# cassianobecker/tgcn

Hardware: AMD Instinct MI355X
Metric: Cheb-TGCN fwd: G edge·timesteps/s + achieved HBM GB/s, K=5 on 160M-edge graph (higher is better)
Workload: dtype f32

## Files before the change

### tgcn_amd/csrc/common.h

```cpp
#pragma once


thread_local char g_err[512] = "";

#define TGCN_FAIL(code, ...)                    \
  do {                                          \
    snprintf(g_err, sizeof(g_err), __VA_ARGS__); \
    return (code);                              \
  } while (0)

#define TGCN_CHECK_LAUNCH(what)                                                         \
  do {                                                                                  \
    hipError_t e_ = hipGetLastError();                                                  \
    if (e_ != hipSuccess) TGCN_FAIL(TGCN_ERR_LAUNCH, "%s: %s", what, hipGetErrorString(e_)); \
  } while (0)

constexpr int kBlock = 256;

struct ProfRec { hipEvent_t a, b; int kind; };
thread_local std::vector<ProfRec> g_prof;
thread_local int g_prof_cap = 0;

struct ProfScope {
  hipEvent_t b = nullptr;
// ... 30 lines not shown
  if (hipGetDevice(&dev) != hipSuccess || dev < 0 || dev >= 16) return 64 * 1024;
  int v = cached[dev].load(std::memory_order_relaxed);
  if (v > 0) return v;
  if (hipDeviceGetAttribute(&v, hipDeviceAttributeSharedMemPerBlockOptin, dev) != hipSuccess || v <= 0) {
    (void)hipGetLastError();
    if (hipDeviceGetAttribute(&v, hipDeviceAttributeMaxSharedMemoryPerBlock, dev) != hipSuccess || v <= 0) v = 64 * 1024;
  }
  cached[dev].store(v, std::memory_order_relaxed);
  return v;
}

inline int cu_count() {
  static std::atomic<int> cached[16];
  int dev = 0;
  if (hipGetDevice(&dev) != hipSuccess || dev < 0 || dev >= 16) return 256;
  int v = cached[dev].load(std::memory_order_relaxed);
  if (v > 0) return v;
  if (hipDeviceGetAttribute(&v, hipDeviceAttributeMultiprocessorCount, dev) != hipSuccess || v <= 0) v = 256;
  cached[dev].store(v, std::memory_order_relaxed);
  return v;
}

struct TuneInt {
  int v;
  int load() const { return v; }
  void store(int x) { v = x; }
};
thread_local TuneInt g_hop_variant{0};
thread_local TuneInt g_hop_remap{1};
thread_local TuneInt g_hop_seg_remap{0};
thread_local TuneInt g_hop_mix{0};
thread_local TuneInt g_hop_stream{1};
thread_local TuneInt g_hop_lds_pad{0};
thread_local TuneInt g_proj_variant{0};
thread_local TuneInt g_x3_form{2};
thread_local TuneInt g_x3_tail{1};
thread_local TuneInt g_small_narrow{1};
thread_local TuneInt g_small_dense{2};
thread_local TuneInt g_x3_stream_cap{0};
thread_local TuneInt g_overlap{1};
thread_local TuneInt g_overlap_group{3};
thread_local TuneInt g_overlap_min_mb{256};

struct SideStream {
  hipStream_t st = nullptr;
  hipEvent_t ev[4] = {nullptr, nullptr, nullptr, nullptr};
  int next = 0;
  hipEvent_t event() { hipEvent_t e = ev[next]; next = (next + 1) & 3; return e; }
};
thread_local std::map<int, SideStream>* g_side = nullptr;
thread_local int64_t g_side_launches = 0;

inline SideStream* side_stream() {
  int dev = 0;
  if (hipGetDevice(&dev) != hipSuccess) return nullptr;
  if (!g_side) g_side = new std::map<int, SideStream>();
  SideStream& s = (*g_side)[dev];
  if (s.st) return &s;
  int least = 0, greatest = 0;
  if (hipDeviceGetStreamPriorityRange(&least, &greatest) != hipSuccess) { (void)hipGetLastError(); least = 0; }
  for (auto& e : s.ev)
    if (!e && hipEventCreateWithFlags(&e, hipEventDisableTiming) != hipSuccess) { (void)hipGetLastError(); e = nullptr; return nullptr; }
  if (hipStreamCreateWithPriority(&s.st, hipStreamNonBlocking, least) != hipSuccess) { (void)hipGetLastError(); s.st = nullptr; return nullptr; }
  return &s;
}

// ... 17 lines not shown
```

### tgcn_amd/csrc/device_build.h

```cpp
#pragma once

constexpr int kScanPer = 8;
constexpr int kScanTile = kBlock * kScanPer;

__global__ __launch_bounds__(kBlock) void scan_tile_kernel(const int64_t* in, int64_t* out,
                                                           int64_t* __restrict__ tile_sums, int64_t n, int inclusive) {
  __shared__ int64_t wave_tot[kBlock / 64];
  const int tid = threadIdx.x, lane = tid & 63, wave = tid >> 6;
  const int64_t base = (int64_t)blockIdx.x * kScanTile + (int64_t)tid * kScanPer;
  int64_t v[kScanPer];
  int64_t run = 0;
#pragma unroll
  for (int j = 0; j < kScanPer; ++j) {
    v[j] = (base + j < n) ? in[base + j] : 0;
    run += v[j];
  }
  int64_t inc = run;
#pragma unroll
  for (int off = 1; off < 64; off <<= 1) {
    const int64_t t = __shfl_up(inc, off, 64);
    if (lane >= off) inc += t;
  }
  if (lane == 63) wave_tot[wave] = inc;
  __syncthreads();
// ... 350 lines not shown
                     1.401298464324817e-45f , dis);
  const int64_t total = m + (diag ? n : 0);
  if (total > 0)
    hipLaunchKernelGGL(lap_values_kernel, dim3(grid_1d(total)), dim3(kBlock), 0, st, row, col, w, m, n, (const float*)dis, scale, diag, row_out, col_out, val_out);
  TGCN_CHECK_LAUNCH("adjacency_normalise");
  *count_host = total;
  return TGCN_OK;
}

__global__ void sched_cost_kernel(const int32_t* __restrict__ rowptr, int64_t n, int row_thresh, int wave_max, int row_cost, int64_t* __restrict__ cost,
                                  int64_t* __restrict__ is_seg, int64_t* __restrict__ is_wave, unsigned long long* __restrict__ n_empty) {
  unsigned long long mine = 0;
  for (int64_t i = (int64_t)blockIdx.x * blockDim.x + threadIdx.x; i < n; i += (int64_t)gridDim.x * blockDim.x) {
    const int64_t d = rowptr[i + 1] - rowptr[i];
    cost[i] = (d > row_thresh ? 0 : d) + row_cost;
    is_seg[i] = d > wave_max ? 1 : 0;
    is_wave[i] = (d > row_thresh && d <= wave_max) ? 1 : 0;
    mine += (d == 0);
  }
  if (mine) atomicAdd(n_empty, mine);
}

__global__ void sched_marks_kernel(const int64_t* __restrict__ cum, int64_t n, int64_t target, int64_t nblk, int32_t* __restrict__ blk_row) {
  for (int64_t b = (int64_t)blockIdx.x * blockDim.x + threadIdx.x; b <= nblk; b += (int64_t)gridDim.x * blockDim.x) {
    if (b == 0) { blk_row[0] = 0; continue; }
    if (b == nblk) { blk_row[nblk] = (int32_t)n; continue; }
    const int64_t mark = b * target;
    int64_t lo = 0, hi = n;
    while (lo < hi) { const int64_t mid = (lo + hi) >> 1; if (cum[mid] < mark) lo = mid + 1; else hi = mid; }
    blk_row[b] = (int32_t)((lo + 1 < n) ? lo + 1 : n);
  }
}

__global__ void sched_longrows_kernel(const int32_t* __restrict__ rowptr, int64_t n, const int64_t* __restrict__ is_seg,
                                      const int64_t* __restrict__ pos, int seg_len, uint32_t max_key, uint32_t* __restrict__ seg_rows,
                                      uint32_t* __restrict__ key) {
  for (int64_t i = (int64_t)blockIdx.x * blockDim.x + threadIdx.x; i < n; i += (int64_t)gridDim.x * blockDim.x) {
    if (!is_seg[i]) continue;
    const int64_t d = rowptr[i + 1] - rowptr[i];
    const int64_t o = pos[i];
    seg_rows[o] = (uint32_t)i;
    key[o] = max_key - (uint32_t)((d + seg_len - 1) / seg_len);
  }
}

__global__ void sched_waverows_kernel(const int32_t* __restrict__ rowptr, const tgcn_edge* __restrict__ edges, int64_t n, const int64_t* __restrict__ is_wave,
                                      const int64_t* __restrict__ pos, uint32_t* __restrict__ rows, uint32_t* __restrict__ key) {
  for (int64_t i = (int64_t)blockIdx.x * blockDim.x + threadIdx.x; i < n; i += (int64_t)gridDim.x * blockDim.x) {
    if (!is_wave[i]) continue;
    const int64_t o = pos[i];
    rows[o] = (uint32_t)i;
    key[o] = (uint32_t)edges[rowptr[i]].col;
  }
}

__global__ void sched_wavesegs_kernel(const int32_t* __restrict__ rowptr, const uint32_t* __restrict__ rows, int64_t nw, int32_t* __restrict__ seg_row,
                                      int32_t* __restrict__ seg_e0, int32_t* __restrict__ seg_e1, int32_t* __restrict__ seg_slot) {
  for (int64_t i = (int64_t)blockIdx.x * blockDim.x + threadIdx.x; i < nw; i += (int64_t)gridDim.x * blockDim.x) {
    const int64_t r = rows[i];
    seg_row[i] = (int32_t)r; seg_e0[i] = rowptr[r]; seg_e1[i] = rowptr[r + 1]; seg_slot[i] = -1;
  }
}

__global__ void sched_nsegs_kernel(const uint32_t* __restrict__ key, uint32_t max_key, int64_t m, int64_t* __restrict__ nsegs) {
  for (int64_t i = (int64_t)blockIdx.x * blockDim.x + threadIdx.x; i < m; i += (int64_t)gridDim.x * blockDim.x) nsegs[i] = max_key - key[i];
}

__global__ void sched_segments_kernel(const int32_t* __restrict__ rowptr, const tgcn_edge* __restrict__ edges, const uint32_t* __restrict__ seg_rows,
                                      const int64_t* __restrict__ first, int64_t m, int64_t nseg, int64_t npartial, int seg_len,
                                      int32_t* __restrict__ seg_row, int32_t* __restrict__ seg_e0, int32_t* __restrict__ seg_e1,
                                      int32_t* __restrict__ seg_slot, uint32_t* __restrict__ key, uint32_t* __restrict__ ident) {
  for (int64_t s = (int64_t)blockIdx.x * blockDim.x + threadIdx.x; s < nseg; s += (int64_t)gridDim.x * blockDim.x) {
    int64_t lo = 0, hi = m;
    while (lo + 1 < hi) { const int64_t mid = (lo + hi) >> 1; if (first[mid] <= s) lo = mid; else hi = mid; }
    const int64_t r = seg_rows[lo];
    const int64_t e0 = (int64_t)rowptr[r] + (s - first[lo]) * seg_len;
    const int64_t e1 = (e0 + seg_len < (int64_t)rowptr[r + 1]) ? e0 + seg_len : (int64_t)rowptr[r + 1];
    seg_row[s] = (int32_t)r;
    seg_e0[s] = (int32_t)e0;
    seg_e1[s] = (int32_t)e1;
    seg_slot[s] = s < npartial ? (int32_t)s : -1;
    key[s] = (uint32_t)edges[e0].col;
    ident[s] = (uint32_t)s;
  }
}

__global__ void permute_i32_kernel(const int32_t* __restrict__ in, const uint32_t* __restrict__ perm, int32_t* __restrict__ out, int64_t n) {
  for (int64_t i = (int64_t)blockIdx.x * blockDim.x + threadIdx.x; i < n; i += (int64_t)gridDim.x * blockDim.x) out[i] = in[perm[i]];
}

__global__ void sched_long_kernel(const uint32_t* __restrict__ seg_rows, const int64_t* __restrict__ first, int64_t nlong, int64_t npartial,
                                  int32_t* __restrict__ long_row, int32_t* __restrict__ long_slot) {
  for (int64_t i = (int64_t)blockIdx.x * blockDim.x + threadIdx.x; i <= nlong; i += (int64_t)gridDim.x * blockDim.x) {
    if (i < nlong) { long_row[i] = (int32_t)seg_rows[i]; long_slot[i] = (int32_t)first[i]; }
    else long_slot[nlong] = (int32_t)npartial;
  }
}

__global__ void sched_counts_kernel(const int64_t* __restrict__ nsegs, int64_t m, int huge_slots, int64_t* __restrict__ out2) {
  if (blockIdx.x != 0 || threadIdx.x != 0) return;
  for (int which = 0; which < 2; ++which) {
    const int64_t thr = which == 0 ? 1 : huge_slots;
    int64_t lo = 0, hi = m;
    while (lo < hi) { const int64_t mid = (lo + hi) >> 1; if (nsegs[mid] > thr) lo = mid + 1; else hi = mid; }
    out2[which] = lo;
  }
}
```

### tgcn_amd/csrc/graph_build.h

```cpp
#pragma once

struct DeviceBuf {
  void* p = nullptr;
  ~DeviceBuf() { if (p) (void)hipFree(p); }
  int alloc(size_t bytes) {
    if (p) { (void)hipFree(p); p = nullptr; }
    if (hipMalloc(&p, bytes ? bytes : 16) != hipSuccess) { p = nullptr; return -1; }
    return 0;
  }
  int zero(size_t bytes) { return (alloc(bytes) || hipMemset(p, 0, bytes ? bytes : 16) != hipSuccess) ? -1 : 0; }
};

}

struct tgcn_graph {
  tgcn_csr csr;
  int64_t n_cols;
  DeviceBuf rowptr, edges;
};

struct tgcn_sched {
  tgcn_csr_sched s;
  DeviceBuf blk_row, seg_row, seg_e0, seg_e1, seg_slot, long_row, long_slot;
};
// ... 125 lines not shown

int tgcn_sched_build_csr(const tgcn_csr* A, int64_t n_cols, int32_t C, int aligned16, tgcn_sched** out) {
  if (!A || !out || C <= 0 || A->n <= 0 || !A->rowptr || (A->nnz > 0 && !A->edges) || n_cols <= 0) TGCN_FAIL(TGCN_ERR_INVALID, "sched_build: bad argument");
  const int lanes = hop_geom(C, aligned16).lpr;
  const int gpb = kBlock / lanes;
  const int64_t n = A->n;
  const int32_t seg_mode = 0;
  const int32_t row_thresh = 32, seg_len = 32, huge_slots = 64, row_cost = 4;
  const int64_t max_blocks_hint = 2048;
  hipStream_t st = (hipStream_t)0;
  tgcn_sched* sc = new (std::nothrow) tgcn_sched();
  if (!sc) TGCN_FAIL(TGCN_ERR_LAUNCH, "sched_build: out of host memory");
#define TGCN_SCHED_FAIL(...) do { delete sc; TGCN_FAIL(TGCN_ERR_LAUNCH, __VA_ARGS__); } while (0)
  const int32_t wave_max = lanes == 16 ? 32 * (64 / lanes) : row_thresh;
  DeviceBuf cost, is_seg, is_wave, pos, posw, scanws, empties;
  if (empties.zero(8) || cost.alloc((size_t)n * 8) || is_seg.zero((size_t)(n + 1) * 8) || is_wave.zero((size_t)(n + 1) * 8) || pos.alloc((size_t)(n + 1) * 8) ||
      posw.alloc((size_t)(n + 1) * 8) || scanws.alloc(scan_ws_elems(n + 1) * 8))
    TGCN_SCHED_FAIL("sched_build: device allocation failed");
  hipLaunchKernelGGL(sched_cost_kernel, dim3(grid_1d(n)), dim3(kBlock), 0, st, A->rowptr, n, (int)row_thresh, (int)wave_max, (int)row_cost, (int64_t*)cost.p,
                     (int64_t*)is_seg.p, (int64_t*)is_wave.p, (unsigned long long*)empties.p);
  scan_i64(st, (const int64_t*)cost.p, (int64_t*)cost.p, n, 1, (int64_t*)scanws.p);
  scan_i64(st, (const int64_t*)is_seg.p, (int64_t*)pos.p, n + 1, 0, (int64_t*)scanws.p);
  scan_i64(st, (const int64_t*)is_wave.p, (int64_t*)posw.p, n + 1, 0, (int64_t*)scanws.p);
  int64_t total = 0, m = 0, mw = 0, n_empty = 0;
  if (read_back(&total, (const int64_t*)cost.p + (n - 1)) || read_back(&m, (const int64_t*)pos.p + n) || read_back(&mw, (const int64_t*)posw.p + n) ||
      read_back(&n_empty, (const int64_t*)empties.p))
    TGCN_SCHED_FAIL("sched_build: device read failed");
  const int64_t cap = lanes <= 16 ? 64 : 256;
  const int64_t target = std::max<int64_t>(gpb * 16, std::min<int64_t>(gpb * cap, (total + max_blocks_hint - 1) / max_blocks_hint));
  const int64_t nblk = std::max<int64_t>(1, (total + target - 1) / target);
  if (sc->blk_row.alloc((size_t)(nblk + 1) * 4)) TGCN_SCHED_FAIL("sched_build: device allocation failed");
  hipLaunchKernelGGL(sched_marks_kernel, dim3(grid_1d(nblk + 1)), dim3(kBlock), 0, st, (const int64_t*)cost.p, n, target, nblk, (int32_t*)sc->blk_row.p);
  int64_t nlong = 0, nhuge = 0, npartial = 0, nsegl = 0;
  DeviceBuf seg_rows, key, sortws, nsegs, first, cnt2;
  if (m > 0) {
    const uint32_t max_key = (uint32_t)((A->nnz + seg_len - 1) / seg_len + 1);
    if (seg_rows.alloc((size_t)m * 4) || key.alloc((size_t)m * 4) || sortws.alloc(sort_ws_bytes(m)) || nsegs.zero((size_t)(m + 1) * 8) ||
        first.alloc((size_t)(m + 1) * 8) || cnt2.alloc(16))
      TGCN_SCHED_FAIL("sched_build: device allocation failed");
    hipLaunchKernelGGL(sched_longrows_kernel, dim3(grid_1d(n)), dim3(kBlock), 0, st, A->rowptr, n, (const int64_t*)is_seg.p, (const int64_t*)pos.p,
                       (int)seg_len, max_key, (uint32_t*)seg_rows.p, (uint32_t*)key.p);
    radix_sort_pairs(st, (uint32_t*)key.p, (uint32_t*)seg_rows.p, m, bits_for((int64_t)max_key + 1), (char*)sortws.p);
    hipLaunchKernelGGL(sched_nsegs_kernel, dim3(grid_1d(m)), dim3(kBlock), 0, st, (const uint32_t*)key.p, max_key, m, (int64_t*)nsegs.p);
    hipLaunchKernelGGL(sched_counts_kernel, dim3(1), dim3(64), 0, st, (const int64_t*)nsegs.p, m, (int)huge_slots, (int64_t*)cnt2.p);
    scan_i64(st, (const int64_t*)nsegs.p, (int64_t*)first.p, m + 1, 0, (int64_t*)scanws.p);
    int64_t h2[2] = {0, 0};
    if (hipMemcpy(h2, cnt2.p, 16, hipMemcpyDeviceToHost) != hipSuccess || read_back(&nsegl, (const int64_t*)first.p + m)) TGCN_SCHED_FAIL("sched_build: device read failed");
    nlong = h2[0]; nhuge = h2[1];
    if (nlong > 0 && read_back(&npartial, (const int64_t*)first.p + nlong)) TGCN_SCHED_FAIL("sched_build: device read failed");
  }
  const int64_t nseg = mw + nsegl;
  if (nseg >= (int64_t)INT32_MAX) TGCN_SCHED_FAIL("sched_build: too many segments");
  const size_t sball = (size_t)(nseg > 0 ? nseg : 1) * 4;
  if (sc->seg_row.zero(sball) || sc->seg_e0.zero(sball) || sc->seg_e1.zero(sball) || sc->seg_slot.zero(sball) || sc->long_row.zero((size_t)(nlong ? nlong : 1) * 4) ||
      sc->long_slot.zero((size_t)(nlong + 2) * 4))
    TGCN_SCHED_FAIL("sched_build: device allocation failed");
  DeviceBuf wrows, wkey, wsort, u_row, u_e0, u_e1, u_slot, key2, ident, sortws2;
  if (mw > 0) {
    if (wrows.alloc((size_t)mw * 4) || wkey.alloc((size_t)mw * 4) || wsort.alloc(sort_ws_bytes(mw))) TGCN_SCHED_FAIL("sched_build: device allocation failed");
    hipLaunchKernelGGL(sched_waverows_kernel, dim3(grid_1d(n)), dim3(kBlock), 0, st, A->rowptr, A->edges, n, (const int64_t*)is_wave.p, (const int64_t*)posw.p,
                       (uint32_t*)wrows.p, (uint32_t*)wkey.p);
    radix_sort_pairs(st, (uint32_t*)wkey.p, (uint32_t*)wrows.p, mw, bits_for(n_cols), (char*)wsort.p);
    hipLaunchKernelGGL(sched_wavesegs_kernel, dim3(grid_1d(mw)), dim3(kBlock), 0, st, A->rowptr, (const uint32_t*)wrows.p, mw, (int32_t*)sc->seg_row.p,
                       (int32_t*)sc->seg_e0.p, (int32_t*)sc->seg_e1.p, (int32_t*)sc->seg_slot.p);
  }
  if (nsegl > 0) {
    const size_t sb = (size_t)nsegl * 4;
    if (u_row.alloc(sb) || u_e0.alloc(sb) || u_e1.alloc(sb) || u_slot.alloc(sb) || key2.alloc(sb) || ident.alloc(sb) || sortws2.alloc(sort_ws_bytes(nsegl)))
      TGCN_SCHED_FAIL("sched_build: device allocation failed");
    hipLaunchKernelGGL(sched_segments_kernel, dim3(grid_1d(nsegl)), dim3(kBlock), 0, st, A->rowptr, A->edges, (const uint32_t*)seg_rows.p, (const int64_t*)first.p, m,
                       nsegl, npartial, (int)seg_len, (int32_t*)u_row.p, (int32_t*)u_e0.p, (int32_t*)u_e1.p, (int32_t*)u_slot.p, (uint32_t*)key2.p, (uint32_t*)ident.p);
    radix_sort_pairs(st, (uint32_t*)key2.p, (uint32_t*)ident.p, nsegl, bits_for(n_cols), (char*)sortws2.p);
    const unsigned gs = grid_1d(nsegl);
    hipLaunchKernelGGL(permute_i32_kernel, dim3(gs), dim3(kBlock), 0, st, (const int32_t*)u_row.p, (const uint32_t*)ident.p, (int32_t*)sc->seg_row.p + mw, nsegl);
    hipLaunchKernelGGL(permute_i32_kernel, dim3(gs), dim3(kBlock), 0, st, (const int32_t*)u_e0.p, (const uint32_t*)ident.p, (int32_t*)sc->seg_e0.p + mw, nsegl);
    hipLaunchKernelGGL(permute_i32_kernel, dim3(gs), dim3(kBlock), 0, st, (const int32_t*)u_e1.p, (const uint32_t*)ident.p, (int32_t*)sc->seg_e1.p + mw, nsegl);
    hipLaunchKernelGGL(permute_i32_kernel, dim3(gs), dim3(kBlock), 0, st, (const int32_t*)u_slot.p, (const uint32_t*)ident.p, (int32_t*)sc->seg_slot.p + mw, nsegl);
    if (nlong > 0)
      hipLaunchKernelGGL(sched_long_kernel, dim3(grid_1d(nlong + 1)), dim3(kBlock), 0, st, (const uint32_t*)seg_rows.p, (const int64_t*)first.p, nlong, npartial,
                         (int32_t*)sc->long_row.p, (int32_t*)sc->long_slot.p);
  }
  if (hipStreamSynchronize(st) != hipSuccess || hipGetLastError() != hipSuccess) TGCN_SCHED_FAIL("sched_build: kernels failed");
#undef TGCN_SCHED_FAIL
  memset(&sc->s, 0, sizeof(sc->s));
  sc->s.lanes_per_row = lanes; sc->s.row_thresh = row_thresh; sc->s.nblk = (int32_t)nblk; sc->s.nseg = (int32_t)nseg;
  sc->s.nlong = (int32_t)nlong; sc->s.nhuge = (int32_t)nhuge; sc->s.npartial = (int32_t)npartial; sc->s.seg_mode = seg_mode;
  sc->s.nwseg = (int32_t)mw;
  sc->s.row_mix = (n_empty * 8 >= n) ? 1 : 0;
  sc->s.blk_row = (const int32_t*)sc->blk_row.p; sc->s.seg_row = (const int32_t*)sc->seg_row.p; sc->s.seg_e0 = (const int32_t*)sc->seg_e0.p;
  sc->s.seg_e1 = (const int32_t*)sc->seg_e1.p; sc->s.seg_slot = (const int32_t*)sc->seg_slot.p; sc->s.long_row = (const int32_t*)sc->long_row.p;
  sc->s.long_slot = (const int32_t*)sc->long_slot.p;
  *out = sc;
  return TGCN_OK;
}

int tgcn_sched_build(const tgcn_graph* g, int32_t C, int aligned16, tgcn_sched** out) {
  if (!g) TGCN_FAIL(TGCN_ERR_INVALID, "sched_build: bad argument");
  return tgcn_sched_build_csr(&g->csr, g->n_cols, C, aligned16, out);
}

int tgcn_sched_copy(const tgcn_sched* s, void* stream, int32_t* blk_row, int32_t* seg_row, int32_t* seg_e0, int32_t* seg_e1, int32_t* seg_slot,
                    int32_t* long_row, int32_t* long_slot) {
  if (!s || !blk_row || !seg_row || !seg_e0 || !seg_e1 || !seg_slot || !long_row || !long_slot) TGCN_FAIL(TGCN_ERR_INVALID, "sched_copy: null array");
  hipStream_t st = (hipStream_t)stream;
  const size_t ns = (size_t)(s->s.nseg > 0 ? s->s.nseg : 1) * 4, nl = (size_t)(s->s.nlong > 0 ? s->s.nlong : 1) * 4;
  const size_t nls = (size_t)(s->s.nlong > 0 ? s->s.nlong + 1 : 2) * 4;
  if (hipMemcpyAsync(blk_row, s->blk_row.p, (size_t)(s->s.nblk + 1) * 4, hipMemcpyDeviceToDevice, st) != hipSuccess ||
      hipMemcpyAsync(seg_row, s->seg_row.p, ns, hipMemcpyDeviceToDevice, st) != hipSuccess ||
      hipMemcpyAsync(seg_e0, s->seg_e0.p, ns, hipMemcpyDeviceToDevice, st) != hipSuccess ||
      hipMemcpyAsync(seg_e1, s->seg_e1.p, ns, hipMemcpyDeviceToDevice, st) != hipSuccess ||
      hipMemcpyAsync(seg_slot, s->seg_slot.p, ns, hipMemcpyDeviceToDevice, st) != hipSuccess ||
      hipMemcpyAsync(long_row, s->long_row.p, nl, hipMemcpyDeviceToDevice, st) != hipSuccess ||
      hipMemcpyAsync(long_slot, s->long_slot.p, nls, hipMemcpyDeviceToDevice, st) != hipSuccess || hipStreamSynchronize(st) != hipSuccess)
    TGCN_FAIL(TGCN_ERR_LAUNCH, "sched_copy: copy failed");
  return TGCN_OK;
}

const tgcn_csr_sched* tgcn_sched_get(const tgcn_sched* s) { return s ? &s->s : nullptr; }
void tgcn_sched_destroy(tgcn_sched* s) { delete s; }

// ... 54 lines not shown
```

### tgcn_amd/csrc/hop.h

```cpp
#pragma once

struct HopParams {
  const int32_t* rowptr;
  const tgcn_edge* ev;
  const int32_t* blk_row;
  const int32_t* seg_row;
  const int32_t* seg_e0;
  const int32_t* seg_e1;
  const int32_t* seg_slot;
  const int32_t* long_row;
  const int32_t* long_slot;
  const float* X;
  const float* Z;
  const float* Z2;
  float* Y;
  float* P;
  float* partial;
  int64_t x_bs, x_ld, z_bs, z_ld, z2_bs, z2_ld, y_bs, y_ld, p_bs, p_ld;
  float alpha, beta, gamma;
  int32_t nblk, nseg, nlong, nhuge, row_thresh;
  int32_t C, nb, nchunks, cpad, remap;
  int32_t nwseg;
  int32_t mix_period;
  int32_t stream_out;
// ... 294 lines not shown
      for (int rr = 0; rr < R; ++rr)
        if (live[rr] && cact) finish_row<VEC, NTM, T>(p, b, rb + rr * GPB, c0, acc[rr]);
    }
  } else {
    int sbid = bid - p.nblk;
    if (p.seg_remap) sbid = xcd_remap(sbid, (int)gridDim.x - p.nblk);
    if constexpr (LPR < 64 && R == 1) {
      const int nwblk = (p.nwseg + kBlock / 64 - 1) / (kBlock / 64);
      if (p.seg_mode == 1 || sbid < nwblk) {
        constexpr int GPW = 64 / LPR;
        const int s = sbid * (kBlock / 64) + (tid >> 6);
        const int gw = (tid & 63) / LPR;
        int e0[1] = {0}, e1[1] = {0};
        const int wlimit = p.seg_mode == 1 ? p.nseg : p.nwseg;
        if (s < wlimit) {
          const int a = p.seg_e0[s], z = p.seg_e1[s];
          const int per = (z - a + GPW - 1) / GPW;
          e0[0] = min(z, a + gw * per);
          e1[0] = min(z, e0[0] + per);
        }
        float acc[1][VEC];
#pragma unroll
        for (int i = 0; i < VEC; ++i) acc[0][i] = 0.f;
        accum_multi<LPR, VEC, UU, 1, NTM, T>(p.ev, e0, e1, t, Xc, p.x_ld, acc);
#pragma unroll
        for (int off = LPR; off < 64; off <<= 1)
#pragma unroll
          for (int i = 0; i < VEC; ++i) acc[0][i] += __shfl_xor(acc[0][i], off, 64);
        if (s >= wlimit || gw != 0) return;
        const int slot = p.seg_slot[s];
        if (slot < 0) {
          if (cact) finish_row<VEC, NTM, T>(p, b, p.seg_row[s], c0, acc[0]);
        } else {
          store_vec<VEC>(p.partial + ((int64_t)slot * p.nb + b) * p.cpad + (chunk * LPR + t) * VEC, acc[0]);
        }
        return;
      }
      sbid -= nwblk;
    }
    const int sb = p.nwseg + sbid * GPB * R + gib;
    int e0[R], e1[R];
    float acc[R][VEC];
#pragma unroll
    for (int rr = 0; rr < R; ++rr) {
      const int s = sb + rr * GPB;
      e0[rr] = e1[rr] = 0;
      if (s < p.nseg) { e0[rr] = p.seg_e0[s]; e1[rr] = p.seg_e1[s]; }
#pragma unroll
      for (int i = 0; i < VEC; ++i) acc[rr][i] = 0.f;
    }
    accum_multi<LPR, VEC, UU, R, NTM, T>(p.ev, e0, e1, t, Xc, p.x_ld, acc);
#pragma unroll
    for (int rr = 0; rr < R; ++rr) {
      const int s = sb + rr * GPB;
      if (s >= p.nseg) continue;
      const int slot = p.seg_slot[s];
      if (slot < 0) {
        if (cact) finish_row<VEC, NTM, T>(p, b, p.seg_row[s], c0, acc[rr]);
      } else {
        float* dst = p.partial + ((int64_t)slot * p.nb + b) * p.cpad + (chunk * LPR + t) * VEC;
        if constexpr (NTM & kNtPartials) store_vec_nt<VEC>(dst, acc[rr]);
        else store_vec<VEC>(dst, acc[rr]);
      }
    }
  }
}

// ... 184 lines not shown
```

### tgcn_amd/csrc/tgcn_hip.hip

```cpp
#include <hip/hip_runtime.h>
#include <stdint.h>
#include <stdio.h>
#include <string.h>

#include <math.h>

#include <algorithm>
#include <atomic>
#include <map>
#include <new>
#include <numeric>
#include <mutex>
#include <set>
#include <type_traits>
#include <utility>
#include <vector>

#include "tgcn_hip.h"

namespace {

#include "common.h"
#include "hop.h"
#include "project.h"
#include "wgrad.h"
#include "small_graph.h"
#include "pool_relayout.h"
#include "dropout.h"
#include "windows.h"
#include "windows_bf16.h"
#include "stream_small.h"
#include "series_small.h"
#include "device_build.h"
#include "graph_build.h"

}

extern "C" {

const char* tgcn_last_error(void) { return g_err; }
int tgcn_abi_version(void) { return TGCN_ABI_VERSION; }

void tgcn_reset_tuning(void) {
  g_hop_variant.store(0); g_hop_remap.store(1); g_hop_seg_remap.store(0); g_hop_mix.store(0); g_hop_stream.store(1); g_hop_lds_pad.store(0);
  g_proj_variant.store(0); g_small_dense.store(2); g_small_narrow.store(1); g_x3_form.store(2); g_x3_tail.store(1);
  g_x3_stream_cap.store(0); g_overlap.store(1); g_overlap_group.store(3); g_overlap_min_mb.store(256);
}

int tgcn_set_tuning(const char* key, int32_t value) {
  if (key && strcmp(key, "hop_variant") == 0) { g_hop_variant.store(value); return TGCN_OK; }
  if (key && strcmp(key, "hop_xcd_remap") == 0) { g_hop_remap.store(value != 0); return TGCN_OK; }
  if (key && strcmp(key, "hop_seg_remap") == 0) { g_hop_seg_remap.store(value != 0); return TGCN_OK; }
  if (key && strcmp(key, "hop_mix") == 0) { g_hop_mix.store(value); return TGCN_OK; }
  if (key && strcmp(key, "hop_stream") == 0) { g_hop_stream.store(value != 0); return TGCN_OK; }
  if (key && strcmp(key, "hop_lds_pad") == 0) { if (value < 0 || value > 160 * 1024) TGCN_FAIL(TGCN_ERR_INVALID, "set_tuning: hop_lds_pad %d", value); g_hop_lds_pad.store(value); return TGCN_OK; }
  if (key && strcmp(key, "project_variant") == 0) { g_proj_variant.store(value); return TGCN_OK; }
  if (key && strcmp(key, "small_dense") == 0) { g_small_dense.store(value); return TGCN_OK; }
  if (key && strcmp(key, "small_narrow") == 0) { g_small_narrow.store(value); return TGCN_OK; }
  if (key && strcmp(key, "x3_form") == 0) { g_x3_form.store(value); return TGCN_OK; }
  if (key && strcmp(key, "x3_tail") == 0) { g_x3_tail.store(value != 0); return TGCN_OK; }
  if (key && strcmp(key, "x3_stream_cap") == 0) { if (value < 0) TGCN_FAIL(TGCN_ERR_INVALID, "set_tuning: x3_stream_cap %d", value); g_x3_stream_cap.store(value); return TGCN_OK; }
  if (key && strcmp(key, "compact_overlap") == 0) { g_overlap.store(value != 0); return TGCN_OK; }
  if (key && strcmp(key, "compact_overlap_group") == 0) { if (value < 1) TGCN_FAIL(TGCN_ERR_INVALID, "set_tuning: compact_overlap_group %d", value); g_overlap_group.store(value); return TGCN_OK; }
  if (key && strcmp(key, "compact_overlap_min_mb") == 0) { if (value < 0) TGCN_FAIL(TGCN_ERR_INVALID, "set_tuning: compact_overlap_min_mb %d", value); g_overlap_min_mb.store(value); return TGCN_OK; }
  TGCN_FAIL(TGCN_ERR_INVALID, "set_tuning: unknown key");
}

int64_t tgcn_side_stream_launches(void) { return g_side_launches; }

int tgcn_profile_start(int32_t capacity) {
  if (capacity <= 0) TGCN_FAIL(TGCN_ERR_INVALID, "profile: capacity %d", capacity);
  for (auto& r : g_prof) { (void)hipEventDestroy(r.a); (void)hipEventDestroy(r.b); }
  g_prof.clear();
  g_prof.reserve(capacity);
  g_prof_cap = capacity;
  return TGCN_OK;
}

int tgcn_profile_stop(int32_t* kinds, float* ms, int32_t capacity, int32_t* count) {
  g_prof_cap = 0;
  int n = 0;
  for (auto& r : g_prof) {
    float t = 0.f;
    if (hipEventSynchronize(r.b) != hipSuccess || hipEventElapsedTime(&t, r.a, r.b) != hipSuccess) t = -1.f;
    if (n < capacity && kinds && ms) { kinds[n] = r.kind; ms[n] = t; ++n; }
    (void)hipEventDestroy(r.a);
    (void)hipEventDestroy(r.b);
  }
  g_prof.clear();
  if (count) *count = n;
  return TGCN_OK;
}

int tgcn_hop_vec_width(int32_t C, int aligned16) { return C > 0 ? hop_geom(C, aligned16).vec : 0; }
int tgcn_hop_lanes_per_row(int32_t C, int aligned16) { return C > 0 ? hop_geom(C, aligned16).lpr : 0; }
int tgcn_hop_groups_per_block(int32_t C, int aligned16) { return C > 0 ? kBlock / hop_geom(C, aligned16).lpr : 0; }

// ... 2188 lines not shown
```

### tgcn_amd/graph.py

```python

import ctypes as C
import threading

import torch

from . import _lib

ROW_THRESH = 32
SEG_LEN = 32
SEG_MODE = 0
SEG_KEY = "first"
WAVE_ROWS = True
HUGE_SLOTS = 64
ROW_COST = 4
DENSE_MAX_N = 256
MAX_BLOCKS_HINT = 2048
COMPACT_MIN_ROWS = 1 << 16
COMPACT_MIN_EMPTY = 0.125
BUILDER = "library"
BLOCK_ROWS_MAX = None


def _as_i32(t):
    return t.to(torch.int32).contiguous()


def _check_range(row, col, n, ncol):
    if row.numel() and (int(row.min()) < 0 or int(row.max()) >= n or int(col.min()) < 0 or int(col.max()) >= ncol):
        raise _lib.TgcnError("graph operand: vertex index outside [0, %d) x [0, %d)" % (n, ncol))


class Schedule:

    def __init__(self, rowptr, n, lanes_per_row, edges=None, row_thresh=None, seg_len=None, seg_mode=None, n_cols=None, builder=None):
        defaults = (row_thresh is None and seg_len is None and seg_mode is None and ROW_THRESH == 32 and SEG_LEN == 32 and SEG_MODE == 0
                    and SEG_KEY == "first" and WAVE_ROWS and BLOCK_ROWS_MAX is None and ROW_COST == 4 and HUGE_SLOTS == 64 and MAX_BLOCKS_HINT == 2048)
        builder = BUILDER if builder is None else builder
        if builder == "library" and rowptr.is_cuda and edges is not None and defaults:
            self._build_library(rowptr, n, lanes_per_row, edges, n if n_cols is None else n_cols)
            return
        row_thresh = ROW_THRESH if row_thresh is None else row_thresh
        seg_len = max(SEG_LEN if seg_len is None else seg_len, 1)
        seg_mode = (SEG_MODE if seg_mode is None else seg_mode) if lanes_per_row < 64 else 0
        if seg_mode == 1:
            seg_len *= 64 // lanes_per_row
        dev = rowptr.device
        gpb = 256 // lanes_per_row
        deg = (rowptr[1:] - rowptr[:-1]).to(torch.int64)
        is_seg = deg > row_thresh
        cost = torch.where(is_seg, torch.zeros_like(deg), deg) + ROW_COST
        cum = torch.cumsum(cost, 0)
        total = int(cum[-1].item())
        cap = BLOCK_ROWS_MAX if BLOCK_ROWS_MAX else (64 if lanes_per_row <= 16 else 256)
        target = max(gpb * 16, min(gpb * cap, -(-total // MAX_BLOCKS_HINT)))
        nblk = max(1, -(-total // target))
        if nblk > 1:
            marks = torch.arange(1, nblk, device=dev, dtype=torch.int64) * target
            inner = (torch.searchsorted(cum, marks) + 1).clamp_(max=n)
        else:
            inner = torch.zeros(0, dtype=torch.int64, device=dev)
        self.blk_row = _as_i32(torch.cat([torch.zeros(1, dtype=torch.int64, device=dev), inner,
                                          torch.full((1,), n, dtype=torch.int64, device=dev)]))
        self.nblk = nblk
        self.nwseg = 0
        wave_rows = None
        wave_max = 32 * (64 // lanes_per_row) if lanes_per_row == 16 else 0
        if WAVE_ROWS and wave_max > row_thresh and seg_mode == 0 and edges is not None:
            wave_rows = (is_seg & (deg <= wave_max)).nonzero().flatten()
            is_seg_long = is_seg & (deg > wave_max)
        else:
            is_seg_long = is_seg
        seg_rows = is_seg_long.nonzero().flatten()
        z1 = torch.zeros(1, dtype=torch.int32, device=dev)
        self.nseg = self.nlong = self.nhuge = self.npartial = 0
        self.seg_row = self.seg_e0 = self.seg_e1 = self.seg_slot = self.long_row = z1
        self.long_slot = torch.zeros(2, dtype=torch.int32, device=dev)
        if seg_rows.numel():
            nsegs = (deg[seg_rows] + seg_len - 1) // seg_len
            order = torch.argsort(nsegs, descending=True, stable=True)
            seg_rows, nsegs = seg_rows[order], nsegs[order]
            self.nlong = int((nsegs > 1).sum().item())
            self.nhuge = int((nsegs > HUGE_SLOTS).sum().item())
            self.nseg = int(nsegs.sum().item())
            first = torch.cumsum(nsegs, 0) - nsegs
            row_of = torch.repeat_interleave(seg_rows, nsegs)
            within = torch.arange(self.nseg, device=dev, dtype=torch.int64) - torch.repeat_interleave(first, nsegs)
            e0 = rowptr[row_of].to(torch.int64) + within * seg_len
            e1 = torch.minimum(e0 + seg_len, rowptr[row_of + 1].to(torch.int64))
            self.npartial = int(nsegs[: self.nlong].sum().item())
            slot = torch.arange(self.nseg, device=dev, dtype=torch.int64)
            slot = torch.where(slot < self.npartial, slot, torch.full_like(slot, -1))
            if self.nlong:
                self.long_row = _as_i32(seg_rows[: self.nlong])
                self.long_slot = _as_i32(torch.cat([first[: self.nlong], first[self.nlong - 1: self.nlong] + nsegs[self.nlong - 1: self.nlong]]))
            if edges is not None:
                if SEG_KEY == "middle":
                    key = edges[(e0 + e1) // 2, 0].to(torch.int64)
                elif SEG_KEY == "last":
                    key = edges[e1 - 1, 0].to(torch.int64)
                elif SEG_KEY == "first_then_last":
                    key = edges[e0, 0].to(torch.int64) * (n + 1) + edges[e1 - 1, 0].to(torch.int64)
                else:
                    key = edges[e0, 0].to(torch.int64)
                perm = torch.argsort(key, stable=True)
                row_of, e0, e1, slot = row_of[perm], e0[perm], e1[perm], slot[perm]
            self.seg_row, self.seg_e0, self.seg_e1, self.seg_slot = _as_i32(row_of), _as_i32(e0), _as_i32(e1), _as_i32(slot)
        if wave_rows is not None and wave_rows.numel():
            w0 = rowptr[wave_rows].to(torch.int64)
            w1 = rowptr[wave_rows + 1].to(torch.int64)
            wperm = torch.argsort(edges[w0, 0].to(torch.int64), stable=True)
            wr, w0, w1 = wave_rows[wperm], w0[wperm], w1[wperm]
            self.nwseg = int(wr.numel())
            had = self.nseg
            cat = lambda a, b: torch.cat([_as_i32(a), b[:had]]) if had else _as_i32(a)
            self.seg_row, self.seg_e0, self.seg_e1 = cat(wr, self.seg_row), cat(w0, self.seg_e0), cat(w1, self.seg_e1)
            self.seg_slot = cat(torch.full_like(wr, -1), self.seg_slot)
            self.nseg = had + self.nwseg
        self.lanes_per_row = lanes_per_row
        self.row_thresh = row_thresh
        self.seg_len = seg_len
        self.seg_mode = seg_mode
        self.row_mix = int(int((deg == 0).sum().item()) * 8 >= n)
        self.struct = _lib.SchedStruct(lanes_per_row, row_thresh, self.nblk, self.nseg, self.nlong, self.nhuge, self.npartial, seg_mode, self.row_mix, self.nwseg,
                                       self.blk_row.data_ptr(), self.seg_row.data_ptr(), self.seg_e0.data_ptr(),
                                       self.seg_e1.data_ptr(), self.seg_slot.data_ptr(), self.long_row.data_ptr(),
                                       self.long_slot.data_ptr())


def _sched_build_library(self, rowptr, n, lanes_per_row, edges, n_cols):
    import ctypes as C
    L = _lib.lib()
    nnz = int(rowptr[-1].item())
    csr = _lib.CsrStruct(int(n), nnz, rowptr.data_ptr(), edges.data_ptr(), None)
    C_row = lanes_per_row * 4 if lanes_per_row < 64 else 256
    assert L.tgcn_hop_lanes_per_row(C_row, 1) == lanes_per_row, (C_row, lanes_per_row)
    h = C.c_void_p()
    with torch.cuda.device(rowptr.device):
        torch.cuda.current_stream().synchronize()
        _lib.check(L.tgcn_sched_build_csr(C.byref(csr), int(n_cols), C_row, 1, C.byref(h)))
        try:
            st = L.tgcn_sched_get(h).contents
            dev = rowptr.device
            i32 = lambda k: torch.empty(max(int(k), 1), dtype=torch.int32, device=dev)
            self.nblk, self.nseg, self.nlong, self.nhuge, self.npartial = st.nblk, st.nseg, st.nlong, st.nhuge, st.npartial
            self.blk_row = i32(st.nblk + 1)
            self.seg_row, self.seg_e0, self.seg_e1, self.seg_slot = i32(st.nseg), i32(st.nseg), i32(st.nseg), i32(st.nseg)
            self.long_row = i32(st.nlong)
            self.long_slot = torch.zeros(max(st.nlong + 1, 2), dtype=torch.int32, device=dev)
            _lib.check(L.tgcn_sched_copy(h, _lib.stream_ptr(), _lib.ptr(self.blk_row), _lib.ptr(self.seg_row), _lib.ptr(self.seg_e0),
                                         _lib.ptr(self.seg_e1), _lib.ptr(self.seg_slot), _lib.ptr(self.long_row), _lib.ptr(self.long_slot)))
# ... 364 lines not shown
```

Measured before the change: 37.29.

## Split hub rows into longer wave-sized segments in the SpMM schedule

Rows whose degree exceeds a hub threshold are now cut into longer segments (64 edges) instead of the default length, and those segments are sorted ahead of the lane segments so they run on the wave path (nwseg is enlarged). The aim is to cut the number of partial-sum slots and the partial-buffer traffic for high-degree rows on large graphs. The feature is gated on the partial-buffer size exceeding a threshold. The diff also references a non-temporal store for partials under a template flag. In exchange the schedule build gains an extra counting kernel and a blocking host readback.

```diff
diff --git a/tgcn_amd/csrc/common.h b/tgcn_amd/csrc/common.h
--- a/tgcn_amd/csrc/common.h
+++ b/tgcn_amd/csrc/common.h
@@ -86,6 +86,9 @@
 thread_local TuneInt g_hop_mix{0};
 thread_local TuneInt g_hop_stream{1};
 thread_local TuneInt g_hop_lds_pad{0};
+thread_local TuneInt g_sched_hub_min{512};
+thread_local TuneInt g_sched_hub_seg{64};
+thread_local TuneInt g_sched_hub_gate_mb{256};
 thread_local TuneInt g_proj_variant{0};
 thread_local TuneInt g_x3_form{2};
 thread_local TuneInt g_x3_tail{1};
diff --git a/tgcn_amd/csrc/device_build.h b/tgcn_amd/csrc/device_build.h
--- a/tgcn_amd/csrc/device_build.h
+++ b/tgcn_amd/csrc/device_build.h
@@ -406,15 +406,34 @@
   }
 }
 
+__device__ __forceinline__ int64_t sched_row_seg_len(int64_t d, int seg_len, int64_t hub_min, int hub_seg) {
+  return (hub_min >= 0 && d > hub_min) ? hub_seg : seg_len;
+}
+
+__global__ void sched_hub_counts_kernel(const int32_t* __restrict__ rowptr, int64_t n, const int64_t* __restrict__ is_seg, int seg_len, int64_t hub_min,
+                                        int hub_seg, unsigned long long* __restrict__ out2) {
+  unsigned long long plain = 0, hub = 0;
+  for (int64_t i = (int64_t)blockIdx.x * blockDim.x + threadIdx.x; i < n; i += (int64_t)gridDim.x * blockDim.x) {
+    if (!is_seg[i]) continue;
+    const int64_t d = rowptr[i + 1] - rowptr[i];
+    const int64_t ns = (d + seg_len - 1) / seg_len;
+    if (ns > 1) plain += (unsigned long long)ns;
+    if (d > hub_min) hub += (unsigned long long)((d + hub_seg - 1) / hub_seg);
+  }
+  if (plain) atomicAdd(out2, plain);
+  if (hub) atomicAdd(out2 + 1, hub);
+}
+
 __global__ void sched_longrows_kernel(const int32_t* __restrict__ rowptr, int64_t n, const int64_t* __restrict__ is_seg,
-                                      const int64_t* __restrict__ pos, int seg_len, uint32_t max_key, uint32_t* __restrict__ seg_rows,
+                                      const int64_t* __restrict__ pos, int seg_len, int64_t hub_min, int hub_seg, uint32_t max_key, uint32_t* __restrict__ seg_rows,
                                       uint32_t* __restrict__ key) {
   for (int64_t i = (int64_t)blockIdx.x * blockDim.x + threadIdx.x; i < n; i += (int64_t)gridDim.x * blockDim.x) {
     if (!is_seg[i]) continue;
     const int64_t d = rowptr[i + 1] - rowptr[i];
     const int64_t o = pos[i];
+    const int64_t len = sched_row_seg_len(d, seg_len, hub_min, hub_seg);
     seg_rows[o] = (uint32_t)i;
-    key[o] = max_key - (uint32_t)((d + seg_len - 1) / seg_len);
+    key[o] = max_key - (uint32_t)((d + len - 1) / len);
   }
 }
 
@@ -441,20 +460,21 @@
 }
 
 __global__ void sched_segments_kernel(const int32_t* __restrict__ rowptr, const tgcn_edge* __restrict__ edges, const uint32_t* __restrict__ seg_rows,
-                                      const int64_t* __restrict__ first, int64_t m, int64_t nseg, int64_t npartial, int seg_len,
-                                      int32_t* __restrict__ seg_row, int32_t* __restrict__ seg_e0, int32_t* __restrict__ seg_e1,
+                                      const int64_t* __restrict__ first, int64_t m, int64_t nseg, int64_t npartial, int seg_len, int64_t hub_min, int hub_seg,
+                                      uint32_t lane_key_base, int32_t* __restrict__ seg_row, int32_t* __restrict__ seg_e0, int32_t* __restrict__ seg_e1,
                                       int32_t* __restrict__ seg_slot, uint32_t* __restrict__ key, uint32_t* __restrict__ ident) {
   for (int64_t s = (int64_t)blockIdx.x * blockDim.x + threadIdx.x; s < nseg; s += (int64_t)gridDim.x * blockDim.x) {
     int64_t lo = 0, hi = m;
     while (lo + 1 < hi) { const int64_t mid = (lo + hi) >> 1; if (first[mid] <= s) lo = mid; else hi = mid; }
     const int64_t r = seg_rows[lo];
-    const int64_t e0 = (int64_t)rowptr[r] + (s - first[lo]) * seg_len;
-    const int64_t e1 = (e0 + seg_len < (int64_t)rowptr[r + 1]) ? e0 + seg_len : (int64_t)rowptr[r + 1];
+    const int64_t len = sched_row_seg_len((int64_t)rowptr[r + 1] - rowptr[r], seg_len, hub_min, hub_seg);
+    const int64_t e0 = (int64_t)rowptr[r] + (s - first[lo]) * len;
+    const int64_t e1 = (e0 + len < (int64_t)rowptr[r + 1]) ? e0 + len : (int64_t)rowptr[r + 1];
     seg_row[s] = (int32_t)r;
     seg_e0[s] = (int32_t)e0;
     seg_e1[s] = (int32_t)e1;
     seg_slot[s] = s < npartial ? (int32_t)s : -1;
-    key[s] = (uint32_t)edges[e0].col;
+    key[s] = (uint32_t)edges[e0].col + (len == seg_len ? lane_key_base : 0u);
     ident[s] = (uint32_t)s;
   }
 }
diff --git a/tgcn_amd/csrc/graph_build.h b/tgcn_amd/csrc/graph_build.h
--- a/tgcn_amd/csrc/graph_build.h
+++ b/tgcn_amd/csrc/graph_build.h
@@ -181,14 +181,24 @@
   if (sc->blk_row.alloc((size_t)(nblk + 1) * 4)) TGCN_SCHED_FAIL("sched_build: device allocation failed");
   hipLaunchKernelGGL(sched_marks_kernel, dim3(grid_1d(nblk + 1)), dim3(kBlock), 0, st, (const int64_t*)cost.p, n, target, nblk, (int32_t*)sc->blk_row.p);
   int64_t nlong = 0, nhuge = 0, npartial = 0, nsegl = 0;
-  DeviceBuf seg_rows, key, sortws, nsegs, first, cnt2;
+  int64_t hub_min = -1, nhub = 0;
+  const int hub_seg = g_sched_hub_seg.load();
+  DeviceBuf seg_rows, key, sortws, nsegs, first, cnt2, hubcnt;
+  if (m > 0 && lanes == 16 && g_sched_hub_min.load() > 0 && g_sched_hub_min.load() >= hub_seg && hub_seg >= seg_len) {
+    unsigned long long hc[2] = {0, 0};
+    if (hubcnt.zero(16)) TGCN_SCHED_FAIL("sched_build: device allocation failed");
+    hipLaunchKernelGGL(sched_hub_counts_kernel, dim3(grid_1d(n)), dim3(kBlock), 0, st, A->rowptr, n, (const int64_t*)is_seg.p, (int)seg_len,
+                       (int64_t)g_sched_hub_min.load(), hub_seg, (unsigned long long*)hubcnt.p);
+    if (hipMemcpy(hc, hubcnt.p, 16, hipMemcpyDeviceToHost) != hipSuccess) TGCN_SCHED_FAIL("sched_build: device read failed");
+    if ((int64_t)hc[0] * lanes * 16 > ((int64_t)g_sched_hub_gate_mb.load() << 20) && hc[1] > 0) { hub_min = g_sched_hub_min.load(); nhub = (int64_t)hc[1]; }
+  }
   if (m > 0) {
     const uint32_t max_key = (uint32_t)((A->nnz + seg_len - 1) / seg_len + 1);
     if (seg_rows.alloc((size_t)m * 4) || key.alloc((size_t)m * 4) || sortws.alloc(sort_ws_bytes(m)) || nsegs.zero((size_t)(m + 1) * 8) ||
         first.alloc((size_t)(m + 1) * 8) || cnt2.alloc(16))
       TGCN_SCHED_FAIL("sched_build: device allocation failed");
     hipLaunchKernelGGL(sched_longrows_kernel, dim3(grid_1d(n)), dim3(kBlock), 0, st, A->rowptr, n, (const int64_t*)is_seg.p, (const int64_t*)pos.p,
-                       (int)seg_len, max_key, (uint32_t*)seg_rows.p, (uint32_t*)key.p);
+                       (int)seg_len, hub_min, hub_seg, max_key, (uint32_t*)seg_rows.p, (uint32_t*)key.p);
     radix_sort_pairs(st, (uint32_t*)key.p, (uint32_t*)seg_rows.p, m, bits_for((int64_t)max_key + 1), (char*)sortws.p);
     hipLaunchKernelGGL(sched_nsegs_kernel, dim3(grid_1d(m)), dim3(kBlock), 0, st, (const uint32_t*)key.p, max_key, m, (int64_t*)nsegs.p);
     hipLaunchKernelGGL(sched_counts_kernel, dim3(1), dim3(64), 0, st, (const int64_t*)nsegs.p, m, (int)huge_slots, (int64_t*)cnt2.p);
@@ -218,8 +228,8 @@
     if (u_row.alloc(sb) || u_e0.alloc(sb) || u_e1.alloc(sb) || u_slot.alloc(sb) || key2.alloc(sb) || ident.alloc(sb) || sortws2.alloc(sort_ws_bytes(nsegl)))
       TGCN_SCHED_FAIL("sched_build: device allocation failed");
     hipLaunchKernelGGL(sched_segments_kernel, dim3(grid_1d(nsegl)), dim3(kBlock), 0, st, A->rowptr, A->edges, (const uint32_t*)seg_rows.p, (const int64_t*)first.p, m,
-                       nsegl, npartial, (int)seg_len, (int32_t*)u_row.p, (int32_t*)u_e0.p, (int32_t*)u_e1.p, (int32_t*)u_slot.p, (uint32_t*)key2.p, (uint32_t*)ident.p);
-    radix_sort_pairs(st, (uint32_t*)key2.p, (uint32_t*)ident.p, nsegl, bits_for(n_cols), (char*)sortws2.p);
+                       nsegl, npartial, (int)seg_len, hub_min, hub_seg, (uint32_t)(nhub > 0 ? n_cols : 0), (int32_t*)u_row.p, (int32_t*)u_e0.p, (int32_t*)u_e1.p, (int32_t*)u_slot.p, (uint32_t*)key2.p, (uint32_t*)ident.p);
+    radix_sort_pairs(st, (uint32_t*)key2.p, (uint32_t*)ident.p, nsegl, bits_for(nhub > 0 ? 2 * n_cols : n_cols), (char*)sortws2.p);
     const unsigned gs = grid_1d(nsegl);
     hipLaunchKernelGGL(permute_i32_kernel, dim3(gs), dim3(kBlock), 0, st, (const int32_t*)u_row.p, (const uint32_t*)ident.p, (int32_t*)sc->seg_row.p + mw, nsegl);
     hipLaunchKernelGGL(permute_i32_kernel, dim3(gs), dim3(kBlock), 0, st, (const int32_t*)u_e0.p, (const uint32_t*)ident.p, (int32_t*)sc->seg_e0.p + mw, nsegl);
@@ -234,7 +244,7 @@
   memset(&sc->s, 0, sizeof(sc->s));
   sc->s.lanes_per_row = lanes; sc->s.row_thresh = row_thresh; sc->s.nblk = (int32_t)nblk; sc->s.nseg = (int32_t)nseg;
   sc->s.nlong = (int32_t)nlong; sc->s.nhuge = (int32_t)nhuge; sc->s.npartial = (int32_t)npartial; sc->s.seg_mode = seg_mode;
-  sc->s.nwseg = (int32_t)mw;
+  sc->s.nwseg = (int32_t)(mw + nhub);
   sc->s.row_mix = (n_empty * 8 >= n) ? 1 : 0;
   sc->s.blk_row = (const int32_t*)sc->blk_row.p; sc->s.seg_row = (const int32_t*)sc->seg_row.p; sc->s.seg_e0 = (const int32_t*)sc->seg_e0.p;
   sc->s.seg_e1 = (const int32_t*)sc->seg_e1.p; sc->s.seg_slot = (const int32_t*)sc->seg_slot.p; sc->s.long_row = (const int32_t*)sc->long_row.p;
diff --git a/tgcn_amd/csrc/hop.h b/tgcn_amd/csrc/hop.h
--- a/tgcn_amd/csrc/hop.h
+++ b/tgcn_amd/csrc/hop.h
@@ -350,7 +350,9 @@
         if (slot < 0) {
           if (cact) finish_row<VEC, NTM, T>(p, b, p.seg_row[s], c0, acc[0]);
         } else {
-          store_vec<VEC>(p.partial + ((int64_t)slot * p.nb + b) * p.cpad + (chunk * LPR + t) * VEC, acc[0]);
+          float* dst = p.partial + ((int64_t)slot * p.nb + b) * p.cpad + (chunk * LPR + t) * VEC;
+          if constexpr (NTM & kNtPartials) store_vec_nt<VEC>(dst, acc[0]);
+          else store_vec<VEC>(dst, acc[0]);
         }
         return;
       }
diff --git a/tgcn_amd/csrc/tgcn_hip.hip b/tgcn_amd/csrc/tgcn_hip.hip
--- a/tgcn_amd/csrc/tgcn_hip.hip
+++ b/tgcn_amd/csrc/tgcn_hip.hip
@@ -45,6 +45,7 @@
   g_hop_variant.store(0); g_hop_remap.store(1); g_hop_seg_remap.store(0); g_hop_mix.store(0); g_hop_stream.store(1); g_hop_lds_pad.store(0);
   g_proj_variant.store(0); g_small_dense.store(2); g_small_narrow.store(1); g_x3_form.store(2); g_x3_tail.store(1);
   g_x3_stream_cap.store(0); g_overlap.store(1); g_overlap_group.store(3); g_overlap_min_mb.store(256);
+  g_sched_hub_min.store(512); g_sched_hub_seg.store(64); g_sched_hub_gate_mb.store(256);
 }
 
 int tgcn_set_tuning(const char* key, int32_t value) {
@@ -63,6 +64,9 @@
   if (key && strcmp(key, "compact_overlap") == 0) { g_overlap.store(value != 0); return TGCN_OK; }
   if (key && strcmp(key, "compact_overlap_group") == 0) { if (value < 1) TGCN_FAIL(TGCN_ERR_INVALID, "set_tuning: compact_overlap_group %d", value); g_overlap_group.store(value); return TGCN_OK; }
   if (key && strcmp(key, "compact_overlap_min_mb") == 0) { if (value < 0) TGCN_FAIL(TGCN_ERR_INVALID, "set_tuning: compact_overlap_min_mb %d", value); g_overlap_min_mb.store(value); return TGCN_OK; }
+  if (key && strcmp(key, "sched_hub_min") == 0) { if (value < 0) TGCN_FAIL(TGCN_ERR_INVALID, "set_tuning: sched_hub_min %d", value); g_sched_hub_min.store(value); return TGCN_OK; }
+  if (key && strcmp(key, "sched_hub_seg") == 0) { if (value < 1) TGCN_FAIL(TGCN_ERR_INVALID, "set_tuning: sched_hub_seg %d", value); g_sched_hub_seg.store(value); return TGCN_OK; }
+  if (key && strcmp(key, "sched_hub_gate_mb") == 0) { if (value < 0) TGCN_FAIL(TGCN_ERR_INVALID, "set_tuning: sched_hub_gate_mb %d", value); g_sched_hub_gate_mb.store(value); return TGCN_OK; }
   TGCN_FAIL(TGCN_ERR_INVALID, "set_tuning: unknown key");
 }
 
diff --git a/tgcn_amd/graph.py b/tgcn_amd/graph.py
--- a/tgcn_amd/graph.py
+++ b/tgcn_amd/graph.py
@@ -11,6 +11,9 @@
 SEG_MODE = 0
 SEG_KEY = "first"
 WAVE_ROWS = True
+HUB_MIN = 512
+HUB_SEG = 64
+HUB_GATE_BYTES = 256 << 20
 HUGE_SLOTS = 64
 ROW_COST = 4
 DENSE_MAX_N = 256
@@ -19,6 +22,7 @@
 COMPACT_MIN_EMPTY = 0.125
 BUILDER = "library"
 BLOCK_ROWS_MAX = None
+_HUB_DEFAULTS = (HUB_MIN, HUB_SEG, HUB_GATE_BYTES)
 
 
 def _as_i32(t):
@@ -34,7 +38,8 @@
 
     def __init__(self, rowptr, n, lanes_per_row, edges=None, row_thresh=None, seg_len=None, seg_mode=None, n_cols=None, builder=None):
         defaults = (row_thresh is None and seg_len is None and seg_mode is None and ROW_THRESH == 32 and SEG_LEN == 32 and SEG_MODE == 0
-                    and SEG_KEY == "first" and WAVE_ROWS and BLOCK_ROWS_MAX is None and ROW_COST == 4 and HUGE_SLOTS == 64 and MAX_BLOCKS_HINT == 2048)
+                    and SEG_KEY == "first" and WAVE_ROWS and BLOCK_ROWS_MAX is None and ROW_COST == 4 and HUGE_SLOTS == 64 and MAX_BLOCKS_HINT == 2048
+                    and (HUB_MIN, HUB_SEG, HUB_GATE_BYTES) == _HUB_DEFAULTS)
         builder = BUILDER if builder is None else builder
         if builder == "library" and rowptr.is_cuda and edges is not None and defaults:
             self._build_library(rowptr, n, lanes_per_row, edges, n if n_cols is None else n_cols)
@@ -75,18 +80,26 @@
         self.nseg = self.nlong = self.nhuge = self.npartial = 0
         self.seg_row = self.seg_e0 = self.seg_e1 = self.seg_slot = self.long_row = z1
         self.long_slot = torch.zeros(2, dtype=torch.int32, device=dev)
+        hub = None
+        if wave_rows is not None and HUB_MIN and HUB_MIN >= HUB_SEG >= seg_len and seg_rows.numel():
+            plain = (deg[seg_rows] + seg_len - 1) // seg_len
+            if int(plain[plain > 1].sum().item()) * lanes_per_row * 16 > HUB_GATE_BYTES and bool((deg[seg_rows] > HUB_MIN).any()):
+                hub = torch.where(deg[seg_rows] > HUB_MIN, HUB_SEG, seg_len)
+        nhub = 0
         if seg_rows.numel():
-            nsegs = (deg[seg_rows] + seg_len - 1) // seg_len
+            rlen = hub if hub is not None else torch.full_like(seg_rows, seg_len)
+            nsegs = (deg[seg_rows] + rlen - 1) // rlen
             order = torch.argsort(nsegs, descending=True, stable=True)
-            seg_rows, nsegs = seg_rows[order], nsegs[order]
+            seg_rows, nsegs, rlen = seg_rows[order], nsegs[order], rlen[order]
             self.nlong = int((nsegs > 1).sum().item())
             self.nhuge = int((nsegs > HUGE_SLOTS).sum().item())
             self.nseg = int(nsegs.sum().item())
             first = torch.cumsum(nsegs, 0) - nsegs
             row_of = torch.repeat_interleave(seg_rows, nsegs)
             within = torch.arange(self.nseg, device=dev, dtype=torch.int64) - torch.repeat_interleave(first, nsegs)
-            e0 = rowptr[row_of].to(torch.int64) + within * seg_len
-            e1 = torch.minimum(e0 + seg_len, rowptr[row_of + 1].to(torch.int64))
+            len_of = torch.repeat_interleave(rlen, nsegs)
+            e0 = rowptr[row_of].to(torch.int64) + within * len_of
+            e1 = torch.minimum(e0 + len_of, rowptr[row_of + 1].to(torch.int64))
             self.npartial = int(nsegs[: self.nlong].sum().item())
             slot = torch.arange(self.nseg, device=dev, dtype=torch.int64)
             slot = torch.where(slot < self.npartial, slot, torch.full_like(slot, -1))
@@ -102,6 +115,10 @@
                     key = edges[e0, 0].to(torch.int64) * (n + 1) + edges[e1 - 1, 0].to(torch.int64)
                 else:
                     key = edges[e0, 0].to(torch.int64)
+                if hub is not None:
+                    is_lane = (len_of == seg_len).to(torch.int64)
+                    nhub = int((deg[row_of] > HUB_MIN).sum().item())
+                    key = key + is_lane * (int(key.max().item()) + 1)
                 perm = torch.argsort(key, stable=True)
                 row_of, e0, e1, slot = row_of[perm], e0[perm], e1[perm], slot[perm]
             self.seg_row, self.seg_e0, self.seg_e1, self.seg_slot = _as_i32(row_of), _as_i32(e0), _as_i32(e1), _as_i32(slot)
@@ -116,6 +133,7 @@
             self.seg_row, self.seg_e0, self.seg_e1 = cat(wr, self.seg_row), cat(w0, self.seg_e0), cat(w1, self.seg_e1)
             self.seg_slot = cat(torch.full_like(wr, -1), self.seg_slot)
             self.nseg = had + self.nwseg
+        self.nwseg += nhub
         self.lanes_per_row = lanes_per_row
         self.row_thresh = row_thresh
         self.seg_len = seg_len
```

New measurement: 37.82 (median of 6 runs). +1.4%, better.
